# zixinz990/quaternion-mpc

Measured on AMD Instinct MI355X. Metric: MPC QP solves/sec (Go1, 12 forces, N=10), higher is better.
Workload: dtype f64

## Files before the change

quaternion-mpc_amd/csrc/qmpc_device.h:

```cpp
#pragma once

#include <hip/hip_runtime.h>
#include <stdint.h>

#include "../../include/qmpc.h"
#include "qmpc_params_dev.h"

namespace qmpc {

constexpr int kWave = 64;

template <class... Tables>
hipError_t set_max_lds(const Tables&... tables) {
  hipError_t e = hipSuccess;
  auto one = [&e](const auto& table) {
    for (auto k : table)
      if (e == hipSuccess) e = hipFuncSetAttribute(reinterpret_cast<const void*>(k), hipFuncAttributeMaxDynamicSharedMemorySize, 160 * 1024);
  };
  (one(tables), ...);
  return e;
}

constexpr int LD = 16;
constexpr int MAT = 12 * LD;
// ... 12 lines not shown
struct Dim {
  static constexpr int NLEG = NL, NU = 3 * NL, NC = 6 * NL, TU = NL / 4;
  static constexpr int KD = 13 * NU, ROT = 21 * NL;
  static constexpr int C_FOOT = 0, C_GB = 3 * NL, C_WD0 = C_GB + 3, C_CR = C_WD0 + 3, C_CON = C_CR + 18,
                       C_X0 = C_CON + NL;
  static constexpr int REC = 32 + 4 * NL;
  static constexpr int R_FOOT = 19, R_CON = 19 + 3 * NL, R_POS = 19 + 4 * NL, R_QD = R_POS + 9;
};

__host__ __device__ inline Layout make_layout(int N, bool kd_global = false, int nl = 4, bool sl_global = false) {
  Layout L;
  int o = 0;
  auto take = [&](int n) { int r = o; o += n; return r; };
  const int nu = 3 * nl, nc = 6 * nl;
  L.cst = take(nl == 4 ? 64 : 80);
  L.bw0 = take(3 * nu);
  L.refp = take(13);
  L.uref = take(nu);
  L.X = take((N + 1) * 13);
  L.U = take(N * nu);
  L.Xc = take((N + 1) * 13);
  L.dU = take(N * nu);
  if (sl_global) {
    L.S = 0; L.LAM = N * nc; L.DS = 2 * N * nc; L.DLAM = 3 * N * nc; L.RC = 4 * N * nc;
  } else {
    L.S = take(N * nc);
    L.LAM = take(N * nc);
    L.DS = take(N * nc);
    L.DLAM = take(N * nc);
    L.RC = take(N * nc);
  }
  L.AB = take(N * kAB);
  L.XT = take((N + 1) * kXT);
  if (kd_global) {
    L.KD = -1;
    L.ROT = -1;
    L.tile = sl_global ? L.X : L.S;
  } else {
    L.KD = take(N * 13 * nu);
    L.ROT = take(N * 21 * nl);
    o = (o + 1) & ~1;
    L.tile = take(MAT);
  }
  L.total = (o + 1) & ~1;
  return L;
}

enum {
  C_FOOT = 0,
  C_GB = 12,
  C_WD0 = 15,
  C_CR = 18,
  C_CON = 36,
  C_X0 = 40,
};

#define QSYNC() __syncthreads()

__device__ __forceinline__ void mtm_load(const double* X, const double* Y, int lane, d4& acc) {
  const double x0 = X[lane], x1 = X[64 + lane], x2 = X[128 + lane];
  const double y0 = Y[lane], y1 = Y[64 + lane], y2 = Y[128 + lane];
  acc = __builtin_amdgcn_mfma_f64_16x16x4f64(x0, y0, acc, 0, 0, 0);
  acc = __builtin_amdgcn_mfma_f64_16x16x4f64(x1, y1, acc, 0, 0, 0);
  acc = __builtin_amdgcn_mfma_f64_16x16x4f64(x2, y2, acc, 0, 0, 0);
}
__device__ __forceinline__ d4 mtm3(const double X[3], const double Y[3], d4 acc) {
  acc = __builtin_amdgcn_mfma_f64_16x16x4f64(X[0], Y[0], acc, 0, 0, 0);
  acc = __builtin_amdgcn_mfma_f64_16x16x4f64(X[1], Y[1], acc, 0, 0, 0);
  acc = __builtin_amdgcn_mfma_f64_16x16x4f64(X[2], Y[2], acc, 0, 0, 0);
  return acc;
}
__device__ __forceinline__ void mtm(double* C, const double* X, const double* Y, int lane) {
  d4 acc = {0.0, 0.0, 0.0, 0.0};
  mtm_load(X, Y, lane, acc);
  C[lane] = acc[0];
  C[64 + lane] = acc[1];
  C[128 + lane] = acc[2];
}

typedef unsigned u2v __attribute__((ext_vector_type(2)));

template <int CTRL>
__device__ __forceinline__ double dpp_mov(double x) {
  int lo = __double2loint(x), hi = __double2hiint(x);
  lo = __builtin_amdgcn_update_dpp(0, lo, CTRL, 0xF, 0xF, true);
  hi = __builtin_amdgcn_update_dpp(0, hi, CTRL, 0xF, 0xF, true);
  return __hiloint2double(hi, lo);
}
__device__ __forceinline__ void swap16(double x, double& even, double& odd) {
  const u2v lo = __builtin_amdgcn_permlane16_swap((unsigned)__double2loint(x), (unsigned)__double2loint(x), false, false);
  const u2v hi = __builtin_amdgcn_permlane16_swap((unsigned)__double2hiint(x), (unsigned)__double2hiint(x), false, false);
  even = __hiloint2double((int)hi[0], (int)lo[0]);
  odd = __hiloint2double((int)hi[1], (int)lo[1]);
}
__device__ __forceinline__ void swap32(double x, double& lower, double& upper) {
  const u2v lo = __builtin_amdgcn_permlane32_swap((unsigned)__double2loint(x), (unsigned)__double2loint(x), false, false);
  const u2v hi = __builtin_amdgcn_permlane32_swap((unsigned)__double2hiint(x), (unsigned)__double2hiint(x), false, false);
  lower = __hiloint2double((int)hi[0], (int)lo[0]);
  upper = __hiloint2double((int)hi[1], (int)lo[1]);
}
template <int G>
__device__ __forceinline__ double rowgroup_bcast(double x) {
  double ev, od, lo, up;
  swap16(x, ev, od);
  swap32((G & 1) ? od : ev, lo, up);
  return (G & 2) ? up : lo;
}

struct OpMin { __device__ __forceinline__ double operator()(double a, double b) const { return fmin(a, b); } };
struct OpMax { __device__ __forceinline__ double operator()(double a, double b) const { return fmax(a, b); } };
struct OpSum { __device__ __forceinline__ double operator()(double a, double b) const { return a + b; } };
template <class Op>
__device__ __forceinline__ double wave_reduce(double v, Op op) {
  v = op(v, dpp_mov<0xB1>(v));
  v = op(v, dpp_mov<0x4E>(v));
  v = op(v, dpp_mov<0x141>(v));
  v = op(v, dpp_mov<0x140>(v));
  double a, b;
  swap16(v, a, b);
  v = op(a, b);
  swap32(v, a, b);
  return op(a, b);
}
__device__ __forceinline__ double wave_min(double v) { return wave_reduce(v, OpMin()); }
__device__ __forceinline__ double wave_max(double v) { return wave_reduce(v, OpMax()); }
__device__ __forceinline__ double wave_sum(double v) { return wave_reduce(v, OpSum()); }

__device__ __forceinline__ double fast_rcp(double x) {
  double r = __builtin_amdgcn_rcp(x);
  r = fma(fma(-x, r, 1.0), r, r);
  r = fma(fma(-x, r, 1.0), r, r);
  return r;
}

__device__ __forceinline__ double fast_rsqrt(double x) {
  double r = __builtin_amdgcn_rsq(x);
  r = r * fma(-0.5 * x * r, r, 1.5);
  r = r * fma(-0.5 * x * r, r, 1.5);
  return r;
}

template <int J>
__device__ __forceinline__ double row_bcast(double x) {
  int lo = __double2loint(x), hi = __double2hiint(x);
  lo = __builtin_amdgcn_update_dpp(0, lo, 0x150 + J, 0xF, 0xF, true);
  hi = __builtin_amdgcn_update_dpp(0, hi, 0x150 + J, 0xF, 0xF, true);
  return __hiloint2double(hi, lo);
}
__device__ __forceinline__ double read_lane(double x, int l) {
  const int lo = __builtin_amdgcn_readlane(__double2loint(x), l);
  const int hi = __builtin_amdgcn_readlane(__double2hiint(x), l);
  return __hiloint2double(hi, lo);
}

__device__ __forceinline__ void quat_G(const double* q, double G[12]) {
  const double s = q[0], x = q[1], y = q[2], z = q[3];
  G[0] = -x; G[1] = -y;  G[2] = -z;
  G[3] = s;  G[4] = -z;  G[5] = y;
  G[6] = z;  G[7] = s;   G[8] = -x;
  G[9] = -y; G[10] = x;  G[11] = s;
}
__device__ __forceinline__ void quat_Omega(const double* w, double O[16]) {
  const double x = w[0], y = w[1], z = w[2];
  O[0] = 0;  O[1] = -x; O[2] = -y;  O[3] = -z;
  O[4] = x;  O[5] = 0;  O[6] = z;   O[7] = -y;
  O[8] = y;  O[9] = -z; O[10] = 0;  O[11] = x;
  O[12] = z; O[13] = y; O[14] = -x; O[15] = 0;
}

template <int NL, bool LEAN>
struct ModelRegsT {
  double gb[3], wd0[3], rm[LEAN ? 3 * NL : 9 * NL];
  __device__ __forceinline__ void load(const double* cst, const double* bw0) {
    typedef Dim<NL> D;
#pragma unroll
    for (int i = 0; i < 3; ++i) { gb[i] = cst[D::C_GB + i]; wd0[i] = cst[D::C_WD0 + i]; }
    if (LEAN) {
#pragma unroll
      for (int i = 0; i < 3 * NL; ++i) rm[i] = cst[D::C_CON + i / 3] * cst[D::C_FOOT + i];
    } else {
#pragma unroll
      for (int i = 0; i < 9 * NL; ++i) rm[i] = bw0[i];
    }
  }
};

template <int NL, bool LEAN>
__device__ __forceinline__ void srbd_step(const DevParams& P, const ModelRegsT<NL, LEAN>& M, const double* x,
                                          const double* u, double* xn) {
  double F[3], vd[3], wd[3];
  {
    double f0[2] = {0, 0}, f1[2] = {0, 0}, f2[2] = {0, 0};
#pragma unroll
    for (int l = 0; l < NL; ++l) { f0[l & 1] += u[3 * l]; f1[l & 1] += u[3 * l + 1]; f2[l & 1] += u[3 * l + 2]; }
    F[0] = f0[0] + f0[1]; F[1] = f1[0] + f1[1]; F[2] = f2[0] + f2[1];
    if (LEAN) {
      double t0[2] = {0, 0}, t1[2] = {0, 0}, t2[2] = {0, 0};
#pragma unroll
      for (int l = 0; l < NL; ++l) {
        const double* r = &M.rm[3 * l];
        const double* f = &u[3 * l];
        t0[l & 1] += r[1] * f[2] - r[2] * f[1];
        t1[l & 1] += r[2] * f[0] - r[0] * f[2];
        t2[l & 1] += r[0] * f[1] - r[1] * f[0];
      }
      const double tau[3] = {t0[0] + t0[1], t1[0] + t1[1], t2[0] + t2[1]};
#pragma unroll
      for (int a = 0; a < 3; ++a)
        wd[a] = M.wd0[a] + (P.Iinv[3 * a] * tau[0] + P.Iinv[3 * a + 1] * tau[1] + P.Iinv[3 * a + 2] * tau[2]);
    } else {
#pragma unroll
      for (int a = 0; a < 3; ++a) {
        const double* b = &M.rm[3 * NL * a];
        double s[4] = {M.wd0[a], 0.0, 0.0, 0.0};
#pragma unroll
        for (int j = 0; j < 3 * NL; ++j) s[(j / 3) & 3] += b[j] * u[j];
        wd[a] = (s[0] + s[1]) + (s[2] + s[3]);
      }
    }
  }
#pragma unroll
  for (int a = 0; a < 3; ++a) vd[a] = F[a] * P.inv_mass + M.gb[a];
  double G[12];
  quat_G(&x[3], G);
  double qm[4], wm[3];
#pragma unroll
  for (int r = 0; r < 4; ++r)
    qm[r] = x[3 + r] + P.hh * (0.5 * (G[3 * r] * x[10] + G[3 * r + 1] * x[11] + G[3 * r + 2] * x[12]));
#pragma unroll
  for (int a = 0; a < 3; ++a) wm[a] = x[10 + a] + P.hh * wd[a];
// ... 658 lines not shown
```

quaternion-mpc_amd/csrc/qmpc_wform.h:

```cpp
#pragma once

namespace qmpc {


struct LayoutW {
  int GK, WR, SLW;
};
constexpr int kGK = 27;
template <int NL = 4>
__host__ __device__ inline size_t wform_slice(int N, bool sl_global = false) {
  return ((size_t)N * (13 * 12 + 21 * NL + kGK + (sl_global ? 18 * NL : 0)) + 1 + 1) & ~(size_t)1;
}
template <int NL = 4>
__host__ __device__ inline Layout make_layout_w(int N, LayoutW* W, bool kd_global = false, bool sl_global = false, bool cv = false,
                                                bool full = false) {
  Layout L;
  int o = 0;
  auto take = [&](int n) { int r = o; o += n; return r; };
  constexpr int nu = 3 * NL, nc = 6 * NL, nl = NL;
  L.cst = take(NL == 4 ? 64 : 80);
  L.bw0 = take(3 * nu);
  L.refp = take(13);
  L.uref = take(nu);
  L.X = take((N + 1) * 13);
// ... 185 lines not shown
      const double e22 = d22 - l20 * d02 - l21 * e21;
      const double id2 = fast_rcp(e22);
#pragma unroll
      for (int i = 0; i < 9; ++i) out[i] = T[i];
      out[9] = l10; out[10] = l20; out[11] = l21; out[12] = id0; out[13] = id1; out[14] = id2;
      out[15] = gq[0]; out[16] = gq[1]; out[17] = gq[2];
      double V[18];
#pragma unroll
      for (int i = 0; i < 9; ++i) V[i] = T[i];
      {
        const double* bw = sm + L.bw0 + 3 * l;
#pragma unroll
        for (int a = 0; a < 3; ++a)
#pragma unroll
          for (int b = 0; b < 3; ++b)
            V[9 + 3 * a + b] = bw[D::NU * a] * T[b] + bw[D::NU * a + 1] * T[3 + b] + bw[D::NU * a + 2] * T[6 + b];
        if (MD == WM_CONVEX) {
          const double* Wk = sm + L.CV + 8 * k;
#pragma unroll
          for (int b = 0; b < 3; ++b) {
            const double t3[3] = {V[9 + b], V[12 + b], V[15 + b]};
            double y[3];
            cv_winv_mul(Wk, t3, y);
            V[9 + b] = y[0]; V[12 + b] = y[1]; V[15 + b] = y[2];
          }
        }
      }
      const double y0 = gq[0], y1 = gq[1] - l10 * y0, y2 = gq[2] - l20 * y0 - l21 * y1;
      const double z0 = id0 * y0, z1 = id1 * y1, z2 = id2 * y2;
      double v0[6], v1[6], v2[6];
#pragma unroll
      for (int i = 0; i < 6; ++i) {
        v0[i] = V[3 * i];
        v1[i] = V[3 * i + 1] - l10 * v0[i];
        v2[i] = V[3 * i + 2] - l20 * v0[i] - l21 * v1[i];
        acc[21 + i] = v0[i] * z0 + v1[i] * z1 + v2[i] * z2;
      }
#pragma unroll
      for (int i = 0; i < 6; ++i) {
        const double b0 = id0 * v0[i], b1 = id1 * v1[i], b2 = id2 * v2[i];
#pragma unroll
        for (int j = i; j < 6; ++j) acc[S6I(i, j)] = b0 * v0[j] + b1 * v1[j] + b2 * v2[j];
      }
    }
#pragma unroll
    for (int i = 0; i < kGK; ++i) {
      double v = acc[i];
      v += dpp_mov<0xB1>(v);
      v += dpp_mov<0x4E>(v);
      if (NL == 8) v += dpp_mov<0x141>(v);
      acc[i] = v;
    }
    if (live && l == 0) {
      double* gk = GK + kGK * k;
#pragma unroll
      for (int i = 0; i < kGK; ++i) gk[i] = acc[i];
    }
  }
  QSYNC();
}

template <bool PROF>
__device__ __forceinline__ void tick_dep(Prof<PROF>& prof, int ph, double& a, double& b) {
  if (PROF) {
    asm volatile("s_nop 0" : "+v"(a), "+v"(b));
    prof.tick(ph);
    asm volatile("s_nop 0" : "+v"(a), "+v"(b));
  }
}

template <bool PROF>
__device__ __forceinline__ void tick_dep1(Prof<PROF>& prof, int ph, double& a) {
  if (PROF) {
    asm volatile("s_nop 0" : "+v"(a));
    prof.tick(ph);
    asm volatile("s_nop 0" : "+v"(a));
  }
}

__device__ __forceinline__ d4 mtm2(const double X[2], const double Y[2], d4 acc) {
  acc = __builtin_amdgcn_mfma_f64_16x16x4f64(X[0], Y[0], acc, 0, 0, 0);
  acc = __builtin_amdgcn_mfma_f64_16x16x4f64(X[1], Y[1], acc, 0, 0, 0);
  return acc;
}
struct ColOps {
  double m1c, m2c, keep, hsel;
  __device__ __forceinline__ void init(const DevParams& P, int c) {
    const double m1 = P.h * (P.hh * (1.0 / P.mass)), m2 = P.h * (1.0 / P.mass);
    m1c = (c < 3) ? m1 : 0.0;
    m2c = (c < 3) ? m2 : ((c < 6) ? P.h : 0.0);
    keep = (c >= 3 && c < 6) ? 0.0 : 1.0;
    hsel = (c >= 6 && c < 9) ? P.h : 0.0;
  }
};
constexpr int kZeroSlots = 54;
template <int NL> __host__ __device__ constexpr int kZeroSlotsT() { return NL == 4 ? kZeroSlots : 70; }
struct BwPat {
  ColOps co;
  double Mc[3], Nc[2], qadd[3], sel[3];
  int ix_w, st_w, ix_a, st_a, ix_x[3], st_x[3], ix_g[2], st_g[2], kwo[2], xoffN[3];
  bool c12;
  template <int NL = 4, int MD = WM_QUAT>
  __device__ __forceinline__ void init(const DevParams& P, const Layout& L, int lane) {
    const int N = P.N;
    const int c = lane & 15, g = lane >> 4;
    co.init(P, c);
    const int zs = L.cst + kZeroSlotsT<NL>();
    const bool c35 = (c >= 3 && c < 6), c911 = (c >= 9 && c < 12);
    c12 = c == 12;
    const int abN = L.AB + kAB * (N - 1);
    ix_w = c35 ? abN + 18 + (c - 3) : zs;   st_w = c35 ? kAB : 0;
    ix_a = c35 ? abN + (c - 3) : (c911 ? abN + 9 + (c - 9) : zs);   st_a = (c35 || c911) ? kAB : 0;
    sel[0] = (g == 3) ? 1.0 : 0.0;
    sel[1] = (g == 0) ? 1.0 : 0.0;
    sel[2] = (g == 1) ? 1.0 : 0.0;
    const double m1 = P.h * (P.hh * (1.0 / P.mass)), m2 = P.h * (1.0 / P.mass);
#pragma unroll
    for (int e = 0; e < 3; ++e) {
      const int r = 4 * e + g;
      const bool phi = (r >= 3 && r < 6);
      double v = 0.0;
      if (c < 6) {
        if (r < 3) v = (r == c) ? m1 : 0.0;
        else if (r >= 6 && r < 9) v = (r - 6 == c) ? m2 : 0.0;
        else if (r >= 9) v = (r - 9 == c - 3) ? P.h : 0.0;
      }
      Mc[e] = v;
      if (MD == WM_CONVEX) qadd[e] = (c < 12 && r == c) ? P.Q[cvperm(r < 12 ? r : 0)] : 0.0;
      else qadd[e] = (c < 12 && r == c && !phi) ? P.Q[(r < 3) ? r : r + 1] : 0.0;
      const bool xv = (MD == WM_CONVEX) ? c12 : ((phi && c35) || c12);
      const int xo = c12 ? 9 + r : 3 * (r - 3) + (c - 3);
      xoffN[e] = xv ? xo : -1;
      ix_x[e] = xv ? L.XT + kXT * (N - 1) + xo : zs;
      st_x[e] = xv ? kXT : 0;
    }
#pragma unroll
    for (int e = 0; e < 2; ++e) {
      const int r = 4 * e + g;
      const bool phi = (r >= 3 && r < 6);
      Nc[e] = (r < 3 && c == r + 6) ? P.h : ((phi && r == c) ? -1.0 : 0.0);
      const bool gv = r < 6 && (c < 6 || c12);
      const int go = c12 ? 21 + r : S6I(r < 6 ? r : 0, c < 6 ? c : 0);
      ix_g[e] = gv ? kGK * (N - 1) + go : kGK * N;
      st_g[e] = gv ? kGK : 0;
      kwo[e] = (r < 6 && c < 13) ? 13 * r + c : -1;
    }
  }
};
__device__ __forceinline__ double fma_bcast345(double acc, double x, const double m[3]) {
  asm("s_nop 1\n\t"
      "v_fmac_f64_dpp %0, %1, %2 row_newbcast:3 row_mask:0xf bank_mask:0xf\n\t"
      "v_fmac_f64_dpp %0, %1, %3 row_newbcast:4 row_mask:0xf bank_mask:0xf\n\t"
      "v_fmac_f64_dpp %0, %1, %4 row_newbcast:5 row_mask:0xf bank_mask:0xf"
      : "+v"(acc)
      : "v"(x), "v"(m[0]), "v"(m[1]), "v"(m[2]));
  return acc;
}
__device__ __forceinline__ double times_M(double x, const ColOps& co, const double wt[3]) {
  double r = co.m1c * x;
  r = fma(co.m2c, dpp_mov<0x106>(x), r);
  return fma_bcast345(r, x, wt);
}
__device__ __forceinline__ double times_Abar(double x, const ColOps& co, const double at[3]) {
  double r = co.keep * x;
  r = fma(co.hsel, dpp_mov<0x116>(x), r);
  return fma_bcast345(r, x, at);
}

template <int J0, bool INV = false>
__device__ __forceinline__ void gj6_pair_step(double M[2], double Rr[2], int c, int g, bool& pd, double* Iv = nullptr) {
  constexpr int ej = J0 >> 2, g0 = J0 & 3, g1 = g0 + 1;
  static_assert((J0 & 1) == 0 && J0 < 6, "pivot pairs (0,1), (2,3), (4,5)");
  const int s0 = (g0 << 4) | c, s1 = (g1 << 4) | c;
  const double m0 = __shfl(M[ej], s0), m1 = __shfl(M[ej], s1);
  const double r0 = __shfl(Rr[ej], s0), r1 = __shfl(Rr[ej], s1);
  double i0 = 0.0, i1 = 0.0;
  if (INV) { i0 = __shfl(Iv[ej], s0); i1 = __shfl(Iv[ej], s1); }
  const double a = read_lane(M[ej], (g0 << 4) | J0), b = read_lane(M[ej], (g0 << 4) | (J0 + 1)),
               d = read_lane(M[ej], (g1 << 4) | (J0 + 1));
  const double det = fma(a, d, -(b * b));
  pd = pd && (a > 0.0) && (det > 0.0);
  const double rd = fast_rcp(det);
  const double ia = a * rd, ib = b * rd, id = d * rd;
#pragma unroll
  for (int e = 0; e < 2; ++e) {
    double c0 = row_bcast<J0>(M[e]), c1 = row_bcast<J0 + 1>(M[e]);
    double bm = M[e], br = Rr[e], bi = INV ? Iv[e] : 0.0;
    if (e == ej) {
      const bool p0 = g == g0, p1 = g == g1;
      c0 = p0 ? 1.0 : (p1 ? 0.0 : c0);
      c1 = p1 ? 1.0 : (p0 ? 0.0 : c1);
      if (p0 || p1) { bm = 0.0; br = 0.0; bi = 0.0; }
    }
    const double f0 = fma(ib, c1, -(id * c0)), f1 = fma(ib, c0, -(ia * c1));
    M[e] = fma(f1, m1, fma(f0, m0, bm));
    Rr[e] = fma(f1, r1, fma(f0, r0, br));
    if (INV) Iv[e] = fma(f1, i1, fma(f0, i0, bi));
  }
}

template <bool PROF, bool REFINE = false, int MD = WM_QUAT>
__device__ inline int backward_pass_w(const DevParams& P, const Layout& L, const BwPat& bp, double* sm, double* KD,
                                      const double* GK, int lane, Prof<PROF>& prof, double* y0out = nullptr) {
  const int N = P.N;
  const int c = lane & 15, g = lane >> 4;
  const double wscale = (MD == WM_CONVEX) ? P.h * P.hh : (0.5 * P.hh) * P.h;
  const ColOps& co = bp.co;
  const double* Mc = bp.Mc;
  const double* Nc = bp.Nc;
  const double* qadd = bp.qadd;
  const double* msel = bp.sel;
  const double* nsel = bp.sel;
  const int* xoffN = bp.xoffN;
  const int* kwo = bp.kwo;
  int ix_w = bp.ix_w, ix_a = bp.ix_a, ix_x[3] = {bp.ix_x[0], bp.ix_x[1], bp.ix_x[2]}, ix_g[2] = {bp.ix_g[0], bp.ix_g[1]};
  const bool rowok1 = kwo[1] >= 0;
  double Pf[3];
  {
    const double* XTk = sm + L.XT + kXT * N;
#pragma unroll
    for (int e = 0; e < 3; ++e) Pf[e] = qadd[e] + ((xoffN[e] >= 0) ? XTk[xoffN[e]] : 0.0);
  }
  bool pd = true;
  const d4 z4 = {0.0, 0.0, 0.0, 0.0};
  struct KnotOps { double wt[3], at[3], gr[2], xt[3]; };
  auto load_ops = [&](KnotOps& o) {
#pragma unroll
    for (int t = 0; t < 3; ++t) {
      o.wt[t] = sm[ix_w + 3 * t]; o.at[t] = sm[ix_a + 3 * t]; o.xt[t] = sm[ix_x[t]];
      ix_x[t] -= bp.st_x[t];
    }
    ix_w -= bp.st_w; ix_a -= bp.st_a;
#pragma unroll
    for (int e = 0; e < 2; ++e) { o.gr[e] = GK[ix_g[e]]; ix_g[e] -= bp.st_g[e]; }
  };
  KnotOps ops, opn;
  load_ops(ops);
  for (int k = N - 1; k >= 0; --k) {
    double wt[3], Mf[3], Nf[2], R6f[2];
    const double* at = ops.at;
    const double* Gf = ops.gr;
    const double* xt = ops.xt;
#pragma unroll
    for (int t = 0; t < 3; ++t) wt[t] = wscale * ops.wt[t];
    Mf[0] = fma(msel[0], wt[0], Mc[0]);
    Mf[1] = fma(msel[1], wt[1], fma(msel[2], wt[2], Mc[1]));
    Mf[2] = Mc[2];
    Nf[0] = fma(nsel[0], at[0], Nc[0]);
    Nf[1] = fma(nsel[1], at[1], fma(nsel[2], at[2], Nc[1]));
    R6f[0] = bp.c12 ? ops.gr[0] : 0.0;
    R6f[1] = bp.c12 ? ops.gr[1] : 0.0;
    tick_dep(prof, PH_BUILD, Pf[0], Pf[1]);
    double Yp[2];
    {
      const d4 a = mtm3(Mf, Pf, z4);
      Yp[0] = a[0]; Yp[1] = a[1];
    }
    if (k > 0) load_ops(opn);
    if (y0out && bp.c12) {
      if (g < 4) y0out[6 * k + g] = Yp[0];
      if (g < 2) y0out[6 * k + 4 + g] = Yp[1];
    }
    tick_dep(prof, PH_DRAIN, Yp[0], Yp[1]);
    double S6[2];
    S6[0] = times_M(Yp[0], co, wt);
    S6[1] = times_M(Yp[1], co, wt);
    double Cf[2], Qf[2], Wm[2];
    {
      const d4 ini = {R6f[0], R6f[1], 0.0, 0.0};
      const d4 a = mtm2(Gf, Yp, ini);
      Cf[0] = a[0]; Cf[1] = a[1];
      const d4 b = mtm2(S6, Cf, z4);
      Qf[0] = b[0]; Qf[1] = b[1];
    }
    Wm[0] = S6[0] + times_M(Qf[0], co, wt);
    Wm[1] = S6[1] + times_M(Qf[1], co, wt);
    tick_dep(prof, PH_MFMA, Wm[0], Wm[1]);
    double Iv[2];
    if (REFINE) {
      Iv[0] = (c == g) ? 1.0 : 0.0;
      Iv[1] = (g < 2 && c == 4 + g) ? 1.0 : 0.0;
    }
    double Xf[2];
    gj6_pair_step<0, REFINE>(Wm, Qf, c, g, pd, Iv);
    gj6_pair_step<2, REFINE>(Wm, Qf, c, g, pd, Iv);
    gj6_pair_step<4, REFINE>(Wm, Qf, c, g, pd, Iv);
    Xf[0] = Qf[0];
    Xf[1] = rowok1 ? Qf[1] : 0.0;
    if (REFINE) {
      double nWi[2], T1[2], nr[2], vv[2];
      nWi[0] = Iv[0];
      nWi[1] = (g < 2) ? Iv[1] : 0.0;
      {
        const d4 a = mtm2(S6, Xf, z4);
        T1[0] = a[0]; T1[1] = a[1];
      }
      {
        const d4 ini = {Cf[0] + Xf[0], Cf[1] + Xf[1], 0.0, 0.0};
        const d4 a = mtm2(Gf, T1, ini);
        nr[0] = a[0]; nr[1] = rowok1 ? a[1] : 0.0;
      }
      {
        const d4 a = mtm2(S6, nr, z4);
        vv[0] = a[0]; vv[1] = a[1];
      }
      {
        const d4 ini = {Xf[0], Xf[1], 0.0, 0.0};
        const d4 a = mtm2(nWi, vv, ini);
        Xf[0] = a[0];
        Xf[1] = rowok1 ? a[1] : 0.0;
      }
    }
    tick_dep(prof, PH_SOLVE, Xf[0], Xf[1]);
    double Pi[3];
    {
      const d4 ini = {Pf[0], Pf[1], Pf[2], 0.0};
      const d4 a = mtm2(Yp, Xf, ini);
      Pi[0] = a[0]; Pi[1] = a[1]; Pi[2] = a[2];
    }
    double Zf[2];
    {
      const d4 ini = {Yp[0], Yp[1], 0.0, 0.0};
      const d4 a = mtm2(S6, Xf, ini);
      Zf[0] = a[0]; Zf[1] = a[1];
    }
    double Uf[3];
#pragma unroll
    for (int e = 0; e < 3; ++e) Uf[e] = times_Abar(Pi[e], co, at);
    {
      const d4 ini = {Uf[0] + (qadd[0] + xt[0]), Uf[1] + (qadd[1] + xt[1]), Uf[2] + (qadd[2] + xt[2]), 0.0};
      const d4 a = mtm2(Nf, Uf, ini);
      Pf[0] = a[0]; Pf[1] = a[1]; Pf[2] = a[2];
    }
    {
      double* KDk = KD + 156 * k;
#pragma unroll
      for (int e = 0; e < 2; ++e) {
        if (kwo[e] >= 0) { KDk[kwo[e]] = Xf[e]; KDk[kwo[e] + 78] = Zf[e]; }
      }
    }
    ops = opn;
    tick_dep(prof, PH_PUPD, Pf[0], Pf[1]);
  }
  return !pd;
}

__device__ __forceinline__ void srbd_step_w(const DevParams& P, const double gb[3], const double wd0[3], const double* x,
                                            const double w[6], double* xn) {
  double vd[3], wd[3];
#pragma unroll
  for (int a = 0; a < 3; ++a) { vd[a] = w[a] * P.inv_mass + gb[a]; wd[a] = wd0[a] + w[3 + a]; }
  double G[12];
  quat_G(&x[3], G);
  double qm[4], wm[3];
#pragma unroll
  for (int r = 0; r < 4; ++r)
    qm[r] = x[3 + r] + P.hh * (0.5 * (G[3 * r] * x[10] + G[3 * r + 1] * x[11] + G[3 * r + 2] * x[12]));
#pragma unroll
  for (int a = 0; a < 3; ++a) wm[a] = x[10 + a] + P.hh * wd[a];
  quat_G(qm, G);
#pragma unroll
  for (int a = 0; a < 3; ++a) {
    xn[a] = x[a] + P.h * (x[7 + a] + P.hh * vd[a]);
    xn[7 + a] = x[7 + a] + P.h * vd[a];
    xn[10 + a] = x[10 + a] + P.h * wd[a];
  }
#pragma unroll
  for (int r = 0; r < 4; ++r)
    xn[3 + r] = x[3 + r] + P.h * (0.5 * (G[3 * r] * wm[0] + G[3 * r + 1] * wm[1] + G[3 * r + 2] * wm[2]));
}

template <bool WITH_DU, int NL = 4>
__device__ inline void wrench_from_inputs(const DevParams& P, const Layout& L, const LayoutW& LW, double* sm, int lane) {
  const int N = P.N;
  constexpr int NU = 3 * NL;
  for (int q = lane; q < 6 * N; q += kWave) {
    const int k = q / 6, i = q - 6 * k;
    double u[NU];
#pragma unroll
    for (int j = 0; j < NU; ++j) u[j] = sm[L.U + NU * k + j] + (WITH_DU ? sm[L.dU + NU * k + j] : 0.0);
    const double* b = sm + L.bw0 + ((i >= 3) ? NU * (i - 3) : 0);
    if (NL == 4) {
      double s0 = 0.0, s1 = 0.0, f0 = 0.0, f1 = 0.0;
#pragma unroll
      for (int j = 0; j < 6; ++j) { s0 += b[j] * u[j]; s1 += b[6 + j] * u[6 + j]; }
#pragma unroll
      for (int a = 0; a < 3; ++a) {
        f0 += (i == a) ? u[a] + u[6 + a] : 0.0;
        f1 += (i == a) ? u[3 + a] + u[9 + a] : 0.0;
      }
      sm[LW.WR + q] = (i < 3) ? f0 + f1 : s0 + s1;
    } else {
      double sv[4] = {0.0, 0.0, 0.0, 0.0}, fv[4] = {0.0, 0.0, 0.0, 0.0};
#pragma unroll
      for (int j = 0; j < NU; ++j) sv[j / 6] += b[j] * u[j];
#pragma unroll
      for (int l = 0; l < NL; ++l)
#pragma unroll
        for (int a = 0; a < 3; ++a) fv[l >> 1] += (i == a) ? u[3 * l + a] : 0.0;
      sm[LW.WR + q] = (i < 3) ? (fv[0] + fv[1]) + (fv[2] + fv[3]) : (sv[0] + sv[1]) + (sv[2] + sv[3]);
    }
  }
  QSYNC();
}

template <int NL = 4, int MD = WM_QUAT>
__device__ inline void rollout_scaled_w(const DevParams& P, const Layout& L, const LayoutW& LW, double* sm, double ap, int lane) {
  typedef Dim<NL> D;
  const int N = P.N;
  const double* cst = sm + L.cst;
  for (int i = lane; i < N * D::NU; i += kWave) sm[L.dU + i] *= ap;
  QSYNC();
  wrench_from_inputs<true, NL>(P, L, LW, sm, lane);
  double gb[3], wd0[3];
#pragma unroll
  for (int a = 0; a < 3; ++a) { gb[a] = cst[D::C_GB + a]; wd0[a] = cst[D::C_WD0 + a]; }
  double x[13], xn[13], w[6], wn[6];
#pragma unroll
  for (int i = 0; i < 13; ++i) x[i] = cst[D::C_X0 + i];
#pragma unroll
  for (int i = 0; i < 6; ++i) w[i] = sm[LW.WR + i];
  for (int k = 0; k < N; ++k) {
    const int kn = (k + 1 < N) ? k + 1 : k;
#pragma unroll
// ... 672 lines not shown
```

quaternion-mpc_amd/csrc/qmpc_wform_body.inc:

```
#ifndef QMPC_WNL
#define QMPC_WNL 4
#define QMPC_WNL_DEFAULTED 1
#endif
#ifndef QMPC_WMODEL
#define QMPC_WMODEL WM_QUAT
#define QMPC_WMODEL_DEFAULTED 1
#endif
  constexpr int WNL = QMPC_WNL;
  constexpr int WMT = QMPC_WMODEL;
  typedef typename std::conditional<WMT == WM_CONVEX, ConvexModel, QuatModelT<WNL>>::type WMD;
  typedef Dim<WNL> WD;
  constexpr int NU = WD::NU, NC = WD::NC;
  const int N = P.N;
  constexpr bool KDG = WVAR == 5 || WVAR == 6;
  constexpr bool SLG = WVAR == 6;
  constexpr bool LEAN = WNL == 8 || SLG;
  LayoutW LW;
  const Layout L = make_layout_w<WNL>(N, &LW, KDG, SLG, WMT == WM_CONVEX);
  double* wsb = KDG ? gws + (size_t)wslot * wform_slice<WNL>(N, SLG) : sm;
  double* KD = wsb + L.KD;
  double* ROT = wsb + L.ROT;
  double* GK = wsb + LW.GK;
  double* sl = SLG ? wsb + LW.SLW : sm;
  const void* in = reinterpret_cast<const double*>(in_) + (size_t)b * WD::REC;
// ... 2 lines not shown
  prof.start();
  setup_instance<WMD>(P, L, sm, in, lane, &status);
  if (status != QMPC_OK) {
    if (lane < NU) forces[NU * (size_t)b + lane] = 0.0;
    if (lane == 0 && info) {
      qmpc_info r = {status, 0, 0.0, 0.0, 0.0, 0.0};
      info[b] = r;
    }
    if (traj_u) for (int i = lane; i < N * NU; i += kWave) traj_u[(size_t)b * N * NU + i] = 0.0;
    if (traj_x) for (int i = lane; i < (N + 1) * WMD::NX; i += kWave) traj_x[(size_t)b * (N + 1) * WMD::NX + i] = 0.0;
    return;
  }
  unsigned conmask = 0;
  for (int l = 0; l < WMD::NL; ++l) conmask |= (sm[L.cst + WD::C_CON + l] != 0.0) ? (1u << l) : 0u;
  conmask = __builtin_amdgcn_readfirstlane(conmask);
  if (lane < 10) sm[L.cst + kZeroSlotsT<WNL>() + lane] = 0.0;
  if (lane == 0) GK[kGK * N] = 0.0;
  BwPat bp;
  if (!KDG) bp.init<WNL, WMT>(P, L, lane);
  if (resume) {
    for (int i = lane; i < N * NU; i += kWave) sm[L.U + i] = resume[8 + i];
  } else if (warm_t > 0) {
    if (lane < NU) {
      const bool stance = (conmask >> (lane / 3)) & 1u;
      for (int k = 0; k < N; ++k) {
        const double prev = sm[L.U + ((k + 1 < N) ? k + 1 : k) * NU + lane];
        sm[L.U + k * NU + lane] = !stance ? 0.0 : (prev != 0.0 ? prev : sm[L.uref + lane]);
      }
    }
  } else {
    for (int i = lane; i < N * NU; i += kWave) sm[L.U + i] = sm[L.uref + (i % NU)];
  }
  QSYNC();
  rollout_open<WMD, false>(P, L, sm, lane);
  wrench_from_inputs<false, WNL>(P, L, LW, sm, lane);
  expansions_w<WNL, WMT>(P, L, LW, sm, lane);
  double sl_part = 0.0, rc_part = 0.0;
  unsigned kapbits = 0;
  if (resume) {
    const double rho = resume[0];
    int j = 0;
    for (int i = lane; i < N * NC; i += kWave, ++j) {
      const int row = i % NC, l = row / 6, r = row - 6 * l;
      const double* cr = sm + L.cst + WD::C_CR + 3 * r;
      const double* ur = sm + L.uref + 3 * l;
      double c0 = cr[0] * ur[0] + cr[1] * ur[1] + cr[2] * ur[2];
      if (r == 4) c0 += -P.fz_max * sm[L.cst + WD::C_CON + l];
      const double s0 = fmax(-c0, 1.0);
      const double sraw = resume[8 + N * NU + i], lam = resume[8 + N * NU + N * NC + i];
      const double sv = fabs(sraw), rc = rho * ((resume[5] != 0.0) ? resume[8 + N * NU + 2 * N * NC + i] : (c0 + s0));
      const bool flag = sraw < 0.0;
      sl[L.S + i] = sv;
      sl[L.RC + i] = rc;
      sl[L.LAM + i] = lam;
      if (!LEAN) sl[L.DS + i] = flag ? 1.0 : 0.0;
      if (conmask & (1u << l)) {
        sl_part += sv * lam;
        rc_part = fmax(rc_part, fabs(rc));
        kapbits |= flag ? (1u << j) : 0u;
      }
    }
  } else
  for (int i = lane; i < N * NC; i += kWave) {
    const double c0 = cone_value<WD>(P, L, sm, i);
    const double s0 = fmax(-c0, 1.0);
    const double lam0 = P.mu0 / s0;
    sl[L.S + i] = s0;
    sl[L.RC + i] = c0 + s0;
    sl[L.LAM + i] = lam0;
    if (!LEAN) sl[L.DS + i] = 0.0;
    if (conmask & (1u << ((i % NC) / 6))) {
      sl_part += s0 * lam0;
      rc_part = fmax(rc_part, fabs(c0 + s0));
    }
  }
  QSYNC();
  prof.tick(PH_SETUP);
  const double inv_rows = 1.0 / (double)(6 * N * __popc(conmask));
  const int it_start = resume ? (int)resume[4] + 1 : 1;
  int it = 0, iters = it_start - 1;
  double mu = 0.0, resid = 0.0, last_step = resume ? resume[3] : 1e300, last_ap = resume ? resume[1] : 0.0,
         last_ad = resume ? resume[2] : 0.0;
  status = QMPC_MAX_ITER;
  for (it = it_start; it <= P.iterations_max + 1; ++it) {
    mu = wave_sum(sl_part) * inv_rows;
    resid = wave_max(rc_part);
    if (mu <= P.mu_final && resid <= P.tol_feas && last_step <= P.tol_step) { status = QMPC_OK; break; }
    if (it > P.iterations_max) break;
    double sg = P.sigma;
    const double amin = fmin(last_ap, last_ad);
    if (it > 1 && amin >= 0.99) sg = P.sigma_fast;
    else if (it > 1 && amin < 0.2) sg = fmax(sg, 0.8);
    else if (it > 1 && amin < 0.5) sg = fmax(sg, 0.5);
    const double target = sg * mu;
    prof.tick(PH_MISC);
    prepass_w<false, WNL, WMT, LEAN>(P, L, sm, sl, ROT, GK, target, lane, kapbits);
    prof.tick(PH_PREPASS);
    if (KDG) bp.init<WNL, WMT>(P, L, lane);
    if (backward_pass_w<PROF, false, WMT>(P, L, bp, sm, KD, GK, lane, prof)) { status = QMPC_NOT_PD; break; }
    QSYNC();
    double ap, ad;
    rollout_closed_w<PROF, !KDG, WNL, WMT>(P, L, LW, sm, KD, ROT, lane, prof);
    prof.tick(PH_ROLL);
    {
      double stp_;
      if (recover_directions_w<WNL, WMT, LEAN>(P, L, sm, sl, ROT, target, lane, &ap, &ad, &stp_, kapbits)) { status = QMPC_NOT_PD; break; }
      last_step = stp_;
    }
    last_ap = ap; last_ad = ad;
    prof.tick(PH_DIRS);
    if (LEAN) apply_w<WNL, true>(P, L, sl, ap, ad, conmask, lane, kapbits, sl_part, rc_part, sm, target);
    if (ap < 1.0) rollout_scaled_w<WNL, WMT>(P, L, LW, sm, ap, lane);
    prof.tick(PH_ROLL);
    if (!LEAN) apply_w<WNL, false>(P, L, sl, ap, ad, conmask, lane, kapbits, sl_part, rc_part);
    prof.tick(PH_APPLY);
    for (int i = lane; i < N * NU; i += kWave) sm[L.U + i] += sm[L.dU + i];
    for (int i = lane; i < (N + 1) * 13; i += kWave) sm[L.X + i] = sm[L.Xc + i];
    QSYNC();
    wrench_from_inputs<false, WNL>(P, L, LW, sm, lane);
    prof.tick(PH_MISC);
    expansions_w<WNL, WMT>(P, L, LW, sm, lane);
    prof.tick(PH_EXPAND);
    iters = it;
  }
  if (lane < NU) forces[NU * (size_t)b + lane] = sm[L.U + lane];
  if (traj_u) for (int i = lane; i < N * NU; i += kWave) traj_u[(size_t)b * N * NU + i] = sm[L.U + i];
  if (traj_x)
    for (int i = lane; i < (N + 1) * WMD::NX; i += kWave) {
      if (WMD::NX == 13) {
        traj_x[(size_t)b * (N + 1) * WMD::NX + i] = sm[L.X + i];
      } else {
        const int k_ = i / WMD::NX, j_ = i - WMD::NX * k_;
        traj_x[(size_t)b * (N + 1) * WMD::NX + i] = sm[L.X + 13 * k_ + j_];
      }
    }
  if (info) {
    const double J = cost_plain<WMD>(P, L, sm, lane);
    double viol = 0.0;
    for (int i = lane; i < N * NC; i += kWave) {
      const int l = (i % NC) / 6;
      if (conmask & (1u << l)) viol = fmax(viol, fmax(cone_value<WD>(P, L, sm, i), 0.0));
    }
    viol = wave_max(viol);
    if (lane == 0) {
      qmpc_info r = {status, iters, J, viol, last_step, mu};
      info[b] = r;
    }
  }
  if (PROF && prof_out && lane == 0) {
    prof.tick(PH_MISC);
#pragma unroll
    for (int i = 0; i < PH_COUNT; ++i) prof_out[16 * (size_t)b + i] = prof.t[i];
    prof_out[16 * (size_t)b + 15] = iters;
  }
#ifdef QMPC_WMODEL_DEFAULTED
#undef QMPC_WMODEL
#undef QMPC_WMODEL_DEFAULTED
#endif
#ifdef QMPC_WNL_DEFAULTED
#undef QMPC_WNL
#undef QMPC_WNL_DEFAULTED
#endif
```

Measured before the change: 1.914 million.

## Skip final-iteration expansions, batch DPP FMAs, use 64-bit DPP broadcasts

Moves the convergence check to the end of each interior-point iteration so the last iteration skips the wrench and expansion recomputation. The wrench recompute is also skipped when a scaled rollout has already run. In the backward pass, times_M and times_Abar are batched into interleaved inline-asm DPP FMA sequences, and row broadcasts use a single 64-bit update_dpp. Pivot-row broadcasts now use row-masked DPP with the kept values carried forward, and the next knot's operand loads are split and issued earlier to overlap with compute. The skip logic changes when convergence is checked and relies on the scaled rollout having already refreshed the wrench state.

```diff
diff --git a/quaternion-mpc_amd/csrc/qmpc_device.h b/quaternion-mpc_amd/csrc/qmpc_device.h
--- a/quaternion-mpc_amd/csrc/qmpc_device.h
+++ b/quaternion-mpc_amd/csrc/qmpc_device.h
@@ -118,10 +118,14 @@
 
 template <int CTRL>
 __device__ __forceinline__ double dpp_mov(double x) {
-  int lo = __double2loint(x), hi = __double2hiint(x);
-  lo = __builtin_amdgcn_update_dpp(0, lo, CTRL, 0xF, 0xF, true);
-  hi = __builtin_amdgcn_update_dpp(0, hi, CTRL, 0xF, 0xF, true);
-  return __hiloint2double(hi, lo);
+  if constexpr (CTRL >= 0x150 && CTRL <= 0x15F) {
+    return __builtin_amdgcn_update_dpp(0.0, x, CTRL, 0xF, 0xF, true);
+  } else {
+    int lo = __double2loint(x), hi = __double2hiint(x);
+    lo = __builtin_amdgcn_update_dpp(0, lo, CTRL, 0xF, 0xF, true);
+    hi = __builtin_amdgcn_update_dpp(0, hi, CTRL, 0xF, 0xF, true);
+    return __hiloint2double(hi, lo);
+  }
 }
 __device__ __forceinline__ void swap16(double x, double& even, double& odd) {
   const u2v lo = __builtin_amdgcn_permlane16_swap((unsigned)__double2loint(x), (unsigned)__double2loint(x), false, false);
@@ -178,10 +182,11 @@
 
 template <int J>
 __device__ __forceinline__ double row_bcast(double x) {
-  int lo = __double2loint(x), hi = __double2hiint(x);
-  lo = __builtin_amdgcn_update_dpp(0, lo, 0x150 + J, 0xF, 0xF, true);
-  hi = __builtin_amdgcn_update_dpp(0, hi, 0x150 + J, 0xF, 0xF, true);
-  return __hiloint2double(hi, lo);
+  return dpp_mov<0x150 + J>(x);
+}
+template <int J, int ROWS>
+__device__ __forceinline__ double row_bcast_rows(double x, double keep) {
+  return __builtin_amdgcn_update_dpp(keep, x, 0x150 + J, ROWS, 0xF, false);
 }
 __device__ __forceinline__ double read_lane(double x, int l) {
   const int lo = __builtin_amdgcn_readlane(__double2loint(x), l);
diff --git a/quaternion-mpc_amd/csrc/qmpc_wform.h b/quaternion-mpc_amd/csrc/qmpc_wform.h
--- a/quaternion-mpc_amd/csrc/qmpc_wform.h
+++ b/quaternion-mpc_amd/csrc/qmpc_wform.h
@@ -291,6 +291,16 @@
   acc = __builtin_amdgcn_mfma_f64_16x16x4f64(X[0], Y[0], acc, 0, 0, 0);
   acc = __builtin_amdgcn_mfma_f64_16x16x4f64(X[1], Y[1], acc, 0, 0, 0);
   return acc;
+}
+__device__ __forceinline__ d4 acc_rows(double a, double b) {
+  d4 v;
+  v[0] = a; v[1] = b;
+  return v;
+}
+__device__ __forceinline__ d4 acc_rows(double a, double b, double c) {
+  d4 v;
+  v[0] = a; v[1] = b; v[2] = c;
+  return v;
 }
 struct ColOps {
   double m1c, m2c, keep, hsel;
@@ -356,28 +366,55 @@
     }
   }
 };
-__device__ __forceinline__ double fma_bcast345(double acc, double x, const double m[3]) {
-  asm("s_nop 1\n\t"
-      "v_fmac_f64_dpp %0, %1, %2 row_newbcast:3 row_mask:0xf bank_mask:0xf\n\t"
-      "v_fmac_f64_dpp %0, %1, %3 row_newbcast:4 row_mask:0xf bank_mask:0xf\n\t"
-      "v_fmac_f64_dpp %0, %1, %4 row_newbcast:5 row_mask:0xf bank_mask:0xf"
-      : "+v"(acc)
-      : "v"(x), "v"(m[0]), "v"(m[1]), "v"(m[2]));
-  return acc;
-}
-__device__ __forceinline__ double times_M(double x, const ColOps& co, const double wt[3]) {
-  double r = co.m1c * x;
-  r = fma(co.m2c, dpp_mov<0x106>(x), r);
-  return fma_bcast345(r, x, wt);
-}
-__device__ __forceinline__ double times_Abar(double x, const ColOps& co, const double at[3]) {
-  double r = co.keep * x;
-  r = fma(co.hsel, dpp_mov<0x116>(x), r);
-  return fma_bcast345(r, x, at);
+__device__ __forceinline__ void fma_bcast345_x2(double r[2], const double x[2], const double sh[2], double cs, const double m[3]) {
+  asm("v_fmac_f64 %0, %4, %5\n\t"
+      "v_fmac_f64 %1, %4, %6\n\t"
+      "v_fmac_f64_dpp %0, %2, %7 row_newbcast:3 row_mask:0xf bank_mask:0xf\n\t"
+      "v_fmac_f64_dpp %1, %3, %7 row_newbcast:3 row_mask:0xf bank_mask:0xf\n\t"
+      "v_fmac_f64_dpp %0, %2, %8 row_newbcast:4 row_mask:0xf bank_mask:0xf\n\t"
+      "v_fmac_f64_dpp %1, %3, %8 row_newbcast:4 row_mask:0xf bank_mask:0xf\n\t"
+      "v_fmac_f64_dpp %0, %2, %9 row_newbcast:5 row_mask:0xf bank_mask:0xf\n\t"
+      "v_fmac_f64_dpp %1, %3, %9 row_newbcast:5 row_mask:0xf bank_mask:0xf"
+      : "+v"(r[0]), "+v"(r[1])
+      : "v"(x[0]), "v"(x[1]), "v"(cs), "v"(sh[0]), "v"(sh[1]), "v"(m[0]), "v"(m[1]), "v"(m[2]));
+}
+__device__ __forceinline__ void fma_bcast345_x3(double r[3], const double x[3], const double sh[3], double cs, const double m[3]) {
+  asm("v_fmac_f64 %0, %6, %7\n\t"
+      "v_fmac_f64 %1, %6, %8\n\t"
+      "v_fmac_f64 %2, %6, %9\n\t"
+      "v_fmac_f64_dpp %0, %3, %10 row_newbcast:3 row_mask:0xf bank_mask:0xf\n\t"
+      "v_fmac_f64_dpp %1, %4, %10 row_newbcast:3 row_mask:0xf bank_mask:0xf\n\t"
+      "v_fmac_f64_dpp %2, %5, %10 row_newbcast:3 row_mask:0xf bank_mask:0xf\n\t"
+      "v_fmac_f64_dpp %0, %3, %11 row_newbcast:4 row_mask:0xf bank_mask:0xf\n\t"
+      "v_fmac_f64_dpp %1, %4, %11 row_newbcast:4 row_mask:0xf bank_mask:0xf\n\t"
+      "v_fmac_f64_dpp %2, %5, %11 row_newbcast:4 row_mask:0xf bank_mask:0xf\n\t"
+      "v_fmac_f64_dpp %0, %3, %12 row_newbcast:5 row_mask:0xf bank_mask:0xf\n\t"
+      "v_fmac_f64_dpp %1, %4, %12 row_newbcast:5 row_mask:0xf bank_mask:0xf\n\t"
+      "v_fmac_f64_dpp %2, %5, %12 row_newbcast:5 row_mask:0xf bank_mask:0xf"
+      : "+v"(r[0]), "+v"(r[1]), "+v"(r[2])
+      : "v"(x[0]), "v"(x[1]), "v"(x[2]), "v"(cs), "v"(sh[0]), "v"(sh[1]), "v"(sh[2]), "v"(m[0]), "v"(m[1]), "v"(m[2]));
+}
+__device__ __forceinline__ void times_M(const double x[2], const ColOps& co, const double wt[3], double r[2]) {
+  double sh[2];
+#pragma unroll
+  for (int e = 0; e < 2; ++e) {
+    r[e] = co.m1c * x[e];
+    sh[e] = dpp_mov<0x106>(x[e]);
+  }
+  fma_bcast345_x2(r, x, sh, co.m2c, wt);
+}
+__device__ __forceinline__ void times_Abar(const double x[3], const ColOps& co, const double at[3], double r[3]) {
+  double sh[3];
+#pragma unroll
+  for (int e = 0; e < 3; ++e) {
+    r[e] = co.keep * x[e];
+    sh[e] = dpp_mov<0x116>(x[e]);
+  }
+  fma_bcast345_x3(r, x, sh, co.hsel, at);
 }
 
 template <int J0, bool INV = false>
-__device__ __forceinline__ void gj6_pair_step(double M[2], double Rr[2], int c, int g, bool& pd, double* Iv = nullptr) {
+__device__ __forceinline__ void gj6_pair_step(double M[2], double Rr[2], double pc[2], int c, int g, bool& pd, double* Iv = nullptr) {
   constexpr int ej = J0 >> 2, g0 = J0 & 3, g1 = g0 + 1;
   static_assert((J0 & 1) == 0 && J0 < 6, "pivot pairs (0,1), (2,3), (4,5)");
   const int s0 = (g0 << 4) | c, s1 = (g1 << 4) | c;
@@ -393,13 +430,17 @@
   const double ia = a * rd, ib = b * rd, id = d * rd;
 #pragma unroll
   for (int e = 0; e < 2; ++e) {
-    double c0 = row_bcast<J0>(M[e]), c1 = row_bcast<J0 + 1>(M[e]);
+    double c0, c1;
     double bm = M[e], br = Rr[e], bi = INV ? Iv[e] : 0.0;
     if (e == ej) {
       const bool p0 = g == g0, p1 = g == g1;
-      c0 = p0 ? 1.0 : (p1 ? 0.0 : c0);
-      c1 = p1 ? 1.0 : (p0 ? 0.0 : c1);
+      constexpr int others = 0xF & ~((1 << g0) | (1 << g1));
+      c0 = pc[0] = row_bcast_rows<J0, others>(M[e], pc[0]);
+      c1 = pc[1] = row_bcast_rows<J0 + 1, others>(M[e], pc[1]);
       if (p0 || p1) { bm = 0.0; br = 0.0; bi = 0.0; }
+    } else {
+      c0 = row_bcast<J0>(M[e]);
+      c1 = row_bcast<J0 + 1>(M[e]);
     }
     const double f0 = fma(ib, c1, -(id * c0)), f1 = fma(ib, c0, -(ia * c1));
     M[e] = fma(f1, m1, fma(f0, m0, bm));
@@ -432,58 +473,64 @@
   }
   bool pd = true;
   const d4 z4 = {0.0, 0.0, 0.0, 0.0};
+  double pc01[2] = {(g == 0) ? 1.0 : 0.0, (g == 1) ? 1.0 : 0.0}, pc23[2] = {(g == 2) ? 1.0 : 0.0, (g == 3) ? 1.0 : 0.0};
   struct KnotOps { double wt[3], at[3], gr[2], xt[3]; };
-  auto load_ops = [&](KnotOps& o) {
-#pragma unroll
-    for (int t = 0; t < 3; ++t) {
-      o.wt[t] = sm[ix_w + 3 * t]; o.at[t] = sm[ix_a + 3 * t]; o.xt[t] = sm[ix_x[t]];
-      ix_x[t] -= bp.st_x[t];
-    }
-    ix_w -= bp.st_w; ix_a -= bp.st_a;
+  auto load_head = [&](KnotOps& o) {
+#pragma unroll
+    for (int t = 0; t < 3; ++t) o.wt[t] = sm[ix_w + 3 * t];
+    ix_w -= bp.st_w;
 #pragma unroll
     for (int e = 0; e < 2; ++e) { o.gr[e] = GK[ix_g[e]]; ix_g[e] -= bp.st_g[e]; }
   };
-  KnotOps ops, opn;
-  load_ops(ops);
+  auto load_tail = [&](KnotOps& o) {
+#pragma unroll
+    for (int t = 0; t < 3; ++t) {
+      o.at[t] = sm[ix_a + 3 * t]; o.xt[t] = sm[ix_x[t]];
+      ix_x[t] -= bp.st_x[t];
+    }
+    ix_a -= bp.st_a;
+  };
+  KnotOps ops;
+  load_head(ops);
   for (int k = N - 1; k >= 0; --k) {
     double wt[3], Mf[3], Nf[2], R6f[2];
     const double* at = ops.at;
-    const double* Gf = ops.gr;
     const double* xt = ops.xt;
+    const double Gf[2] = {ops.gr[0], ops.gr[1]};
 #pragma unroll
     for (int t = 0; t < 3; ++t) wt[t] = wscale * ops.wt[t];
+    load_tail(ops);
     Mf[0] = fma(msel[0], wt[0], Mc[0]);
     Mf[1] = fma(msel[1], wt[1], fma(msel[2], wt[2], Mc[1]));
     Mf[2] = Mc[2];
     Nf[0] = fma(nsel[0], at[0], Nc[0]);
     Nf[1] = fma(nsel[1], at[1], fma(nsel[2], at[2], Nc[1]));
-    R6f[0] = bp.c12 ? ops.gr[0] : 0.0;
-    R6f[1] = bp.c12 ? ops.gr[1] : 0.0;
+    R6f[0] = bp.c12 ? Gf[0] : 0.0;
+    R6f[1] = bp.c12 ? Gf[1] : 0.0;
     tick_dep(prof, PH_BUILD, Pf[0], Pf[1]);
     double Yp[2];
     {
       const d4 a = mtm3(Mf, Pf, z4);
       Yp[0] = a[0]; Yp[1] = a[1];
     }
-    if (k > 0) load_ops(opn);
     if (y0out && bp.c12) {
       if (g < 4) y0out[6 * k + g] = Yp[0];
       if (g < 2) y0out[6 * k + 4 + g] = Yp[1];
     }
     tick_dep(prof, PH_DRAIN, Yp[0], Yp[1]);
     double S6[2];
-    S6[0] = times_M(Yp[0], co, wt);
-    S6[1] = times_M(Yp[1], co, wt);
+    times_M(Yp, co, wt, S6);
     double Cf[2], Qf[2], Wm[2];
     {
-      const d4 ini = {R6f[0], R6f[1], 0.0, 0.0};
-      const d4 a = mtm2(Gf, Yp, ini);
+      const d4 a = mtm2(Gf, Yp, acc_rows(R6f[0], R6f[1]));
       Cf[0] = a[0]; Cf[1] = a[1];
       const d4 b = mtm2(S6, Cf, z4);
       Qf[0] = b[0]; Qf[1] = b[1];
     }
-    Wm[0] = S6[0] + times_M(Qf[0], co, wt);
-    Wm[1] = S6[1] + times_M(Qf[1], co, wt);
+    times_M(Qf, co, wt, Wm);
+    Wm[0] = S6[0] + Wm[0];
+    Wm[1] = S6[1] + Wm[1];
+    if (k > 0) load_head(ops);
     tick_dep(prof, PH_MFMA, Wm[0], Wm[1]);
     double Iv[2];
     if (REFINE) {
@@ -491,9 +538,9 @@
       Iv[1] = (g < 2 && c == 4 + g) ? 1.0 : 0.0;
     }
     double Xf[2];
-    gj6_pair_step<0, REFINE>(Wm, Qf, c, g, pd, Iv);
-    gj6_pair_step<2, REFINE>(Wm, Qf, c, g, pd, Iv);
-    gj6_pair_step<4, REFINE>(Wm, Qf, c, g, pd, Iv);
+    gj6_pair_step<0, REFINE>(Wm, Qf, pc01, c, g, pd, Iv);
+    gj6_pair_step<2, REFINE>(Wm, Qf, pc23, c, g, pd, Iv);
+    gj6_pair_step<4, REFINE>(Wm, Qf, pc01, c, g, pd, Iv);
     Xf[0] = Qf[0];
     Xf[1] = rowok1 ? Qf[1] : 0.0;
     if (REFINE) {
@@ -523,22 +570,18 @@
     tick_dep(prof, PH_SOLVE, Xf[0], Xf[1]);
     double Pi[3];
     {
-      const d4 ini = {Pf[0], Pf[1], Pf[2], 0.0};
-      const d4 a = mtm2(Yp, Xf, ini);
+      const d4 a = mtm2(Yp, Xf, acc_rows(Pf[0], Pf[1], Pf[2]));
       Pi[0] = a[0]; Pi[1] = a[1]; Pi[2] = a[2];
     }
     double Zf[2];
     {
-      const d4 ini = {Yp[0], Yp[1], 0.0, 0.0};
-      const d4 a = mtm2(S6, Xf, ini);
+      const d4 a = mtm2(S6, Xf, acc_rows(Yp[0], Yp[1]));
       Zf[0] = a[0]; Zf[1] = a[1];
     }
     double Uf[3];
-#pragma unroll
-    for (int e = 0; e < 3; ++e) Uf[e] = times_Abar(Pi[e], co, at);
+    times_Abar(Pi, co, at, Uf);
     {
-      const d4 ini = {Uf[0] + (qadd[0] + xt[0]), Uf[1] + (qadd[1] + xt[1]), Uf[2] + (qadd[2] + xt[2]), 0.0};
-      const d4 a = mtm2(Nf, Uf, ini);
+      const d4 a = mtm2(Nf, Uf, acc_rows(Uf[0] + (qadd[0] + xt[0]), Uf[1] + (qadd[1] + xt[1]), Uf[2] + (qadd[2] + xt[2])));
       Pf[0] = a[0]; Pf[1] = a[1]; Pf[2] = a[2];
     }
     {
@@ -548,7 +591,6 @@
         if (kwo[e] >= 0) { KDk[kwo[e]] = Xf[e]; KDk[kwo[e] + 78] = Zf[e]; }
       }
     }
-    ops = opn;
     tick_dep(prof, PH_PUPD, Pf[0], Pf[1]);
   }
   return !pd;
diff --git a/quaternion-mpc_amd/csrc/qmpc_wform_body.inc b/quaternion-mpc_amd/csrc/qmpc_wform_body.inc
--- a/quaternion-mpc_amd/csrc/qmpc_wform_body.inc
+++ b/quaternion-mpc_amd/csrc/qmpc_wform_body.inc
@@ -108,9 +108,9 @@
   double mu = 0.0, resid = 0.0, last_step = resume ? resume[3] : 1e300, last_ap = resume ? resume[1] : 0.0,
          last_ad = resume ? resume[2] : 0.0;
   status = QMPC_MAX_ITER;
+  mu = wave_sum(sl_part) * inv_rows;
+  resid = wave_max(rc_part);
   for (it = it_start; it <= P.iterations_max + 1; ++it) {
-    mu = wave_sum(sl_part) * inv_rows;
-    resid = wave_max(rc_part);
     if (mu <= P.mu_final && resid <= P.tol_feas && last_step <= P.tol_step) { status = QMPC_OK; break; }
     if (it > P.iterations_max) break;
     double sg = P.sigma;
@@ -143,11 +143,14 @@
     for (int i = lane; i < N * NU; i += kWave) sm[L.U + i] += sm[L.dU + i];
     for (int i = lane; i < (N + 1) * 13; i += kWave) sm[L.X + i] = sm[L.Xc + i];
     QSYNC();
-    wrench_from_inputs<false, WNL>(P, L, LW, sm, lane);
+    iters = it;
+    mu = wave_sum(sl_part) * inv_rows;
+    resid = wave_max(rc_part);
+    if ((mu <= P.mu_final && resid <= P.tol_feas && last_step <= P.tol_step) || it >= P.iterations_max) continue;
+    if (!(ap < 1.0)) wrench_from_inputs<false, WNL>(P, L, LW, sm, lane);
     prof.tick(PH_MISC);
     expansions_w<WNL, WMT>(P, L, LW, sm, lane);
     prof.tick(PH_EXPAND);
-    iters = it;
   }
   if (lane < NU) forces[NU * (size_t)b + lane] = sm[L.U + lane];
   if (traj_u) for (int i = lane; i < N * NU; i += kWave) traj_u[(size_t)b * N * NU + i] = sm[L.U + i];
```

New measurement: 1.997 million, median of 6. 1.04x the previous value.
